# NeRF-3DTalker/NeRF-3DTalker-code

Hardware: AMD Instinct MI355X
Metric: rendered frames/sec @512^2 x 64 samples/ray (higher is better)
Workload: dtype bf16; 1 GPU; cfg2-R: 16 heads/GPU/step, 64x64 rays x 64 samples -> fused MLP+composite -> neural renderer -> 512x512 RGB (+ background image); rays_per_frame=4096, samples_per_ray=64, parallelism=frames sharded over 1 rank(s), no data-path collective, ranks_seen_by_backend=1

## Files before the change

### include/n3dt.h

```cpp
#ifndef N3DT_API_H_
#define N3DT_API_H_

#include <stddef.h>
#include <stdint.h>

#ifdef __cplusplus
extern "C" {
#endif

#define N3DT_ABI_VERSION 5

#define N3DT_F32 0
#define N3DT_BF16 1
#define N3DT_F16 2
#define N3DT_BF16X3 3

#define N3DT_OK 0
#define N3DT_EINVAL (-1)
#define N3DT_EWORKSPACE (-2)
#define N3DT_EHIP (-3)

#define N3DT_PE_DIM 63
#define N3DT_MLP_LAYERS 12

// ... 76 lines not shown

int n3dt_fine_sample(const N3dtGeom* g, int n_fine, const float* weight, const float* T, const float* t_rand, const float* u,
                     float* z_planes, void* stream);

int n3dt_sample_points(const N3dtGeom* g, const float* xy, const float* R, const float* T, const float* Kinv, const float* t_rand,
                       float* pts, float* zvals, float* z_dists, float* ray_d, float* ray_l, void* stream);
int n3dt_embed(int batch, size_t m, const float* pts, float* pe, void* stream);
int n3dt_embed_freqs(int batch, size_t m, int n_freqs, const float* pts, float* pe, void* stream);
size_t n3dt_mlp_points_workspace_bytes(const N3dtGeom* g, size_t m);
int n3dt_mlp_points(const N3dtGeom* g, size_t m, const N3dtMlpParams* p, const float* audio, const float* embed_vps,
                    const float* embed_vds, float* rgb, float* density, void* workspace, size_t workspace_bytes, void* stream);
int n3dt_composite(int batch, int n_rays, int n_samples, int channels, const float* rgb, const float* density, const float* z_dists,
                   const float* zvals, float* feat, float* bg_alpha, float* depth, float* weight, void* stream);
int n3dt_x16_pack_probe(int precision, int form, size_t n, const float* in, uint16_t* out, void* stream);
int n3dt_x16_pe_probe(int precision, int form, size_t n, const float* points, uint16_t* out, void* stream);

size_t n3dt_neural_render_workspace_bytes(const N3dtGeom* g, int nb);
int n3dt_neural_render_fwd(const N3dtGeom* g, int nb, int precision, const N3dtRenderParams* p, const float* featmap,
                           float* img, void* workspace, size_t workspace_bytes, void* stream);

int n3dt_neural_render_pack(const N3dtGeom* g, int nb, int precision, const N3dtRenderParams* p, void* workspace,
                            size_t workspace_bytes, void* stream);
int n3dt_neural_render_fwd_reuse(const N3dtGeom* g, int nb, int precision, const N3dtRenderParams* p, const float* featmap,
                                 float* img, void* workspace, size_t workspace_bytes, void* stream);
int n3dt_feat_to_rgb0(int nb, int n_pix, const float* featmap, const float* w, const float* b, float* rgb0, void* stream);
int n3dt_neural_render_fwd16_reuse(const N3dtGeom* g, int nb, int precision, const N3dtRenderParams* p, const void* featmap16,
                                   const float* rgb0, float* img, void* workspace, size_t workspace_bytes, void* stream);

size_t n3dt_render_train_saved_bytes(const N3dtGeom* g);
size_t n3dt_render_train_workspace_bytes(const N3dtGeom* g);
// ... 214 lines not shown
```

### nerf-3dtalker-code_amd/csrc/n3dt_api.hip

```cpp
#include <hip/hip_runtime.h>
#include <stdarg.h>
#include <stdio.h>
#include <stdlib.h>
#include <string.h>

#include <mutex>

#include "../../include/n3dt.h"
#include "n3dt_layout.h"
#include "n3dt_launch.h"
#include "eval_metrics_core.h"
#include "lpips_core.h"
#include "mel_core.h"
#include "syncnet_core.h"
#include "wav2lip_core.h"
#include "s3fd_core.h"

static thread_local char g_err[256] = "";

__attribute__((format(printf, 2, 3))) static int failf(int code, const char* fmt, ...) {
    va_list ap;
    va_start(ap, fmt);
    vsnprintf(g_err, sizeof(g_err), fmt, ap);
    va_end(ap);
// ... 258 lines not shown
    if (n < 512 || n % 512 != 0 || n / 512 > 0x7fffffffu) return fail(N3DT_EINVAL, "n3dt_x16_pack_probe: n must be a multiple of 512, at most 2^40");
    if (!in || !out) return fail(N3DT_EINVAL, "n3dt_x16_pack_probe: NULL argument");
    n3dt_launch_x16_pack_probe(precision, form, n, in, out, (hipStream_t)stream);
    return check_hip("n3dt_x16_pack_probe");
}

extern "C" int n3dt_x16_pe_probe(int precision, int form, size_t n, const float* points, uint16_t* out, void* stream) {
    if (precision != N3DT_BF16 && precision != N3DT_F16) return fail(N3DT_EINVAL, "n3dt_x16_pe_probe: precision must be N3DT_BF16 or N3DT_F16");
    if (form != 0 && form != 1) return fail(N3DT_EINVAL, "n3dt_x16_pe_probe: form must be 0 (by octave half) or 1 (per channel)");
    if (n < 32 || n % 32 != 0 || n / 32 > 0x7fffffffu) return fail(N3DT_EINVAL, "n3dt_x16_pe_probe: n must be a multiple of 32, at most 2^36");
    if (!points || !out) return fail(N3DT_EINVAL, "n3dt_x16_pe_probe: NULL argument");
    n3dt_launch_x16_pe_probe(precision, form, n, points, out, (hipStream_t)stream);
    return check_hip("n3dt_x16_pe_probe");
}

extern "C" int n3dt_fine_sample(const N3dtGeom* g, int n_fine, const float* weight, const float* T, const float* t_rand, const float* u,
                                float* z_planes, void* stream) {
    int rc = check_geom(g, N3DT_F32);
    if (rc) return rc;
    if (!weight || !T || !z_planes) return fail(N3DT_EINVAL, "n3dt_fine_sample: NULL argument");
    if (g->z_planes_given && !t_rand) return fail(N3DT_EINVAL, "n3dt_fine_sample: z_planes_given but no coarse planes passed as t_rand");
    if (g->n_samples < 3) return fail(N3DT_EINVAL, "n3dt_fine_sample: needs at least 3 coarse samples");
    if (n_fine < 0 || g->n_samples + n_fine + 1 > 2048) return fail(N3DT_EINVAL, "n3dt_fine_sample: more than 2048 planes per ray");
    n3dt_launch_fine_sample(g, n_fine, weight, T, t_rand, u, z_planes, (hipStream_t)stream);
    return check_hip("n3dt_fine_sample");
}

extern "C" size_t n3dt_neural_render_workspace_bytes(const N3dtGeom* g, int nb) {
    if (!g || nb < 1 || g->n_blocks < 1 || g->n_blocks > N3DT_MAX_BLOCKS || g->featmap_size < 2) return 0;
    return n3dt_nr_workspace_floats(g, nb) * sizeof(float);
// ... 887 lines not shown
```

### nerf-3dtalker-code_amd/csrc/n3dt_launch.h

```cpp
#pragma once
#include <stddef.h>
#include <hip/hip_runtime.h>

#include "../../include/n3dt.h"

struct MelSignal;

extern "C" {
int n3dt_prof_span_begin(hipStream_t s);
void n3dt_prof_span_end(int slot, hipStream_t s);

void n3dt_launch_small_gemm(int M, int N, int K, const float* A, long sam, long sak, const float* B, long sbn, long sbk, float* C, long ldc,
                            int accumulate, hipStream_t s);
void n3dt_launch_pack(const N3dtGeom* g, int precision, const N3dtMlpParams* p, void* packed, hipStream_t stream);
void n3dt_launch_fold(const N3dtGeom* g, const N3dtMlpParams* p, const float* shape, const float* appea, const float* audio, float* fold,
                      int merged_rgb, hipStream_t stream);
void n3dt_launch_rayfold(const N3dtGeom* g, const float* fold, const float* ray_bias, hipStream_t s);
void n3dt_launch_ray_vd_bias(const N3dtGeom* g, const float* w_vd, long ld_w, const float* xy, const float* R, const float* Kinv,
                             float* ray_bias, hipStream_t s);
void n3dt_launch_ray_head(const N3dtGeom* g, int bpr, int bs, const float* part, const float* wlocal, const float* tail,
                          const float* bg_featmap, int bg_hwc, float* fg_feat, float* bg_alpha, float* depth, float* weight,
                          float* merge_feat, hipStream_t stream);
void n3dt_launch_ray_head_mfma(const N3dtGeom* g, int bpr, int bs, const float* part, const float* wlocal, const float* tail,
                               const float* bg_featmap, int bg_hwc, float* fg_feat, float* bg_alpha, float* depth, float* weight,
// ... 20 lines not shown
                                    float* geo, void* gates, hipStream_t stream);
void n3dt_launch_nerf_fwd_x16s(const N3dtGeom* g, const void* packed, const float* fold, const float* xy, const float* R, const float* T,
                               const float* Kinv, const float* t_rand, float* part, float* wlocal, hipStream_t stream);

void n3dt_launch_sample_points(const N3dtGeom* g, const float* xy, const float* R, const float* T, const float* Kinv, const float* t_rand,
                               float* pts, float* zvals, float* z_dists, float* ray_d, float* ray_l, hipStream_t s);
void n3dt_launch_embed(int B, size_t M, const float* pts, float* pe, hipStream_t s);
void n3dt_launch_embed_freqs(int B, size_t M, int n_freqs, const float* pts, float* pe, hipStream_t s);
size_t n3dt_seam_mlp_ws_floats(const N3dtGeom* g, size_t M);
void n3dt_launch_mlp_points(const N3dtGeom* g, size_t M, const N3dtMlpParams* p, const float* audio, const float* vps, const float* vds,
                            float* rgb, float* density, float* ws, hipStream_t s);
void n3dt_launch_composite(int B, int Nr, int Ns, int C, const float* rgb, const float* density, const float* z_dists, const float* zvals,
                           float* feat, float* bg_alpha, float* depth, float* weight, hipStream_t s);
void n3dt_launch_x16_pe_probe(int precision, int form, size_t n, const float* points, unsigned short* out, hipStream_t s);
void n3dt_launch_x16_pack_probe(int precision, int form, size_t n, const float* in, unsigned short* out, hipStream_t s);

size_t n3dt_nr_workspace_floats(const N3dtGeom* g, int nb);
void n3dt_launch_feat_to_rgb0(int nb, int n_pix, const float* featmap, const float* w, const float* b, float* rgb0, hipStream_t s);
void n3dt_launch_neural_render16(const N3dtGeom* g, int nb, int precision, const N3dtRenderParams* p, const void* featmap16,
                                 const float* rgb0, float* img, float* ws, hipStream_t s);
void n3dt_launch_neural_render(const N3dtGeom* g, int nb, int precision, const N3dtRenderParams* p, const float* featmap, float* img,
                               float* ws, int pack_mode, hipStream_t s);
void n3dt_launch_nr_train16_fwd(const N3dtGeom* g, int nb, const N3dtRenderParams* p, const float* featmap, float* img,
                                unsigned char* saved, unsigned char* ws, hipStream_t s);
void n3dt_launch_gemm_regions_bf16(int M, int N, int K, int n_regions, const void* const* base, const int* width, const int* ld,
                                   const float* Wt, const void* gate, void* y, hipStream_t s);
void n3dt_launch_conv1x1_bwd_bf16(int M, int N, int K, const void* dy, const float* Wt, int mode, const void* res, void* y, hipStream_t s);
void n3dt_launch_conv1x1_bf16(int M, int N, int K, const void* x, int x_is_16, const float* Wt, const float* bias, float slope, void* y,
                              hipStream_t s);

// ... 109 lines not shown
```

### nerf-3dtalker-code_amd/csrc/nerf_fwd_x16.hip

```cpp
#include "x16_core.h"
#include "n3dt_launch.h"


#ifndef X16_SAVE_DEPTH
#define X16_SAVE_DEPTH 3
#endif
#ifndef X16_FWD_ISSUE
#define X16_FWD_ISSUE 0, 1, 2
#endif
template <int PREC>
struct X16SaveStage {
    unsigned char* tile0;
    unsigned* gate0;
};

enum { X16_BIAS_GLOBAL_MFMA = 0, X16_BIAS_LDS_MFMA = 1, X16_BIAS_LDS_C = 2 };
#define X16_BIAS_SLOT 1536
struct X16BiasLds {
    unsigned char* slots;
    unsigned addr;
    __device__ __forceinline__ void stage_in(const float* table, const int n, const int slot, const int lane, const int at = 0) const {
#pragma unroll
        for (int i = 0; i < 6; ++i)
            if (64 * i < n)
                __builtin_amdgcn_global_load_lds((const GLOBAL_AS void*)(table + 64 * i + lane),
                                                 (LDS_AS void*)(slots + slot * X16_BIAS_SLOT + 4 * at + 256 * i), 4, 0, 0);
    }
    __device__ __forceinline__ unsigned at(const int slot, const int at = 0) const { return addr + slot * X16_BIAS_SLOT + 4 * at; }
};
struct X16TileInit {
    f32x4 q[2][4];
    template <int SET, int OFF>
    __device__ __forceinline__ void issue(const unsigned table) {
        asm volatile("ds_read_b128 %0, %4 offset:%5\n\tds_read_b128 %1, %4 offset:%6\n\t"
                     "ds_read_b128 %2, %4 offset:%7\n\tds_read_b128 %3, %4 offset:%8"
                     : "=&v"(q[SET][0]), "=&v"(q[SET][1]), "=&v"(q[SET][2]), "=&v"(q[SET][3])
                     : "v"(table), "i"(OFF), "i"(OFF + 32), "i"(OFF + 64), "i"(OFF + 96)
                     : "memory");
    }
    template <int SET>
    __device__ __forceinline__ void landed() {
// ... 31 lines not shown
    [[maybe_unused]] float bias_cur = 0.0f, bias_nxt = 0.0f;
    if constexpr (LB) {
        x16_bias_read<0>(bias_cur, bias_lds);
        asm volatile("s_waitcnt lgkmcnt(0)" : "+v"(bias_cur));
    } else if constexpr (!CINIT) {
        bias_cur = bias[c];
    }
    auto finish_half = [&](const int t, const int half) {
        float v[8];
#pragma unroll
        for (int r = 0; r < 8; ++r) v[r] = acc[8 * half + r];
        frag f = X16<PREC>::pack(v);
        if (MODE == MODE_HIDDEN) f = X16<PREC>::relu(f, relu_lo);
        hout[2 * t + half] = f;
    };
    static_for<0, NT>([&](auto ot_c) {
        constexpr int ot = decltype(ot_c)::value;
        constexpr int cs = (PAR + ot) & 1, ns = cs ^ 1;
        constexpr bool FETCH = CINIT && ot + 1 < NT;
        X16_T(const unsigned long long s0 = x16_now();)
        if constexpr (CINIT) {
            if constexpr (ot == 0) ti.template settle<cs>();
            if constexpr (FETCH) ti.template issue<ns, (ot + 1) * 128>(bias_lds);
            acc = ti.template get<cs>();
        } else {
            const frag bf = X16<PREC>::bias_frag(bias_cur, h == 0);
            if constexpr (LB) {
                if constexpr (ot + 1 < NT) x16_bias_read<(ot + 1) * 128>(bias_nxt, bias_lds);
            } else {
                if (ot + 1 < NT) bias_cur = bias[(ot + 1) * 32 + c];
            }
            f32x16 zero;
#pragma unroll
            for (int r = 0; r < 16; ++r) zero[r] = 0.0f;
            acc = X16<PREC>::mfma(bf, ones, zero);
        }
        X16_T(const unsigned long long s1 = x16_now(); const unsigned long long rv0 = ws.t_rv;)
        static_for<0, KS>([&](auto ks_c) {
            constexpr int ks = decltype(ks_c)::value;
            const frag a_cur = ws.template next<MODE == MODE_COMPOSITE, NT * KS, ot * KS + ks,
                                                (FETCH && ks < WS::depth - 1) ? X16_TILE_INIT_READS : 0>();
            frag b;
            if (ks < KPE) {
                if (pe_lds) b = *reinterpret_cast<const frag*>(pe_lds + ks * X16_PIECE);
                else b = pe_reg[ks < 4 ? ks : 0];
            } else {
                b = hin[ks >= KPE ? ks - KPE : 0];
            }
            acc = X16<PREC>::mfma(a_cur, b, acc);
        });
        if constexpr (FETCH) ti.template landed<ns>();
        else if constexpr (CINIT && NEXT && ot + 1 == NT) ti.template issue<ns, 0>(next_lds);
        if constexpr (LB && ot + 1 < NT) {
            asm volatile("" : "+v"(bias_nxt), "+v"(acc));
            bias_cur = bias_nxt;
        }
        X16_T(const unsigned long long s2 = x16_now();)
        if (PACKS) {
            finish_half(ot, 0);
            finish_half(ot, 1);
        }
        if constexpr (SAVE && PACKS) {
#ifndef X16_DIAG_NOIMG
            x16_image_store<PREC>(hout[2 * ot], hout[2 * ot + 1], sv->tile0 + ot * 2 * X16_PIECE);
// ... 19 lines not shown
            aux = acc[0];
        } else if (MODE == MODE_COMPOSITE) {
#pragma unroll
            for (int r = 0; r < 16; ++r) red[(ot & 1) * 16 + r] = fmaxf(acc[r], 0.0f) * aux;
            if constexpr (SAVE) {
#pragma unroll
                for (int half = 0; half < 2; ++half) {
                    float v[8];
#pragma unroll
                    for (int r = 0; r < 8; ++r) v[r] = fmaxf(acc[8 * half + r], 0.0f);
                    __builtin_nontemporal_store(X16<PREC>::pack(v), reinterpret_cast<frag*>(sv->tile0 + (2 * ot + half) * X16_PIECE));
                }
                ws.note_stores(2);
            }
            if (ot & 1) {
                float s = butterfly32(red, c);
                const int v = ((c & 1) << 4) | ((c & 2) << 2) | (c & 4) | ((c & 8) >> 2) | ((c & 16) >> 4);
                const int reg = v & 15, tile = (ot - 1) + (v >> 4);
                if (live) po[tile * 32 + (reg & 3) + 8 * (reg >> 2) + 4 * h] = s;
            }
        }
        X16_T(const unsigned long long s3 = x16_now(); ws.t_bias += s1 - s0; ws.t_mfma += (s2 - s1) - (ws.t_rv - rv0); ws.t_epi += s3 - s2;
              if (ws.tl && ws.tile_no >= 20 && ws.tile_no < 33 && (threadIdx.x & 63) == 0) {
                  ws.tl[4 + 2 * (ws.tile_no - 20)] = (float)(s1 & 0xFFFFFF);
                  ws.tl[5 + 2 * (ws.tile_no - 20)] = (float)(s2 & 0xFFFFFF);
              }
              ++ws.tile_no;)
    });
}

struct X16TrainSave {
    unsigned char* xT;
    unsigned char* gS;
    float* geo;
    unsigned* gates;
};

template <int PREC, int WAVES, bool SAVE = false>
__device__ __forceinline__ void nerf_fwd_x16_body(
    const N3dtGeom& g, const unsigned char* __restrict__ packed, const float* __restrict__ fold, const float* __restrict__ xy,
    const float* __restrict__ R, const float* __restrict__ T, const float* __restrict__ Kinv, const float* __restrict__ t_rand,
    float* __restrict__ part, float* __restrict__ wlocal, int bpr, long total_blocks, unsigned char* lds, const int wave,
    const X16TrainSave tsv = X16TrainSave{nullptr, nullptr, nullptr, nullptr}) {
    typedef typename X16<PREC>::frag frag;
    const int lane = threadIdx.x & 63;
    const int c = lane & 31, h = lane >> 5;
    X16_T(const unsigned long long t_entry = x16_now();)

    typedef WeightStream<PREC, WAVES, X16_NCHUNK, X16_NBUF, SAVE ? X16_SAVE_DEPTH : X16_DEPTH,
                         std::conditional_t<SAVE, X16Issue<>, X16Issue<X16_FWD_ISSUE>>> WS;
    WS ws;
    if constexpr (SAVE) {
        ws.gsrc = packed + (size_t)wave * WS::PPW * X16_PIECE + lane * 16;
    } else {
        ws.gsrc = packed + (size_t)wave * WS::PPW * X16_PIECE;
        ws.voff = lane * 16;
    }
    ws.ring = lds;
    ws.lds_addr0 = (unsigned)(size_t)(LDS_AS unsigned char*)lds + lane * 16;
// ... 31 lines not shown
    auto sv_hidden = [&](const int l) -> const X16SaveStage<PREC>* {
        if constexpr (SAVE) {
            svs.tile0 = xT_blk + (size_t)(2 + 12 * l) * 2 * X16_PIECE;
            svs.gate0 = tsv.gates + ((size_t)rec * 8 + l) * 6 * 64 + lane;
            return &svs;
        } else {
            return nullptr;
        }
    };
    constexpr int BIAS = SAVE ? X16_BIAS_LDS_MFMA : X16_BIAS_LDS_C;
    constexpr int BIAS_DEN = BIAS == X16_BIAS_LDS_C ? X16_BIAS_LDS_C : X16_BIAS_GLOBAL_MFMA;
    X16BiasLds bl{nullptr, 0u};
    constexpr int DEN_AT = 192;
    bl.slots = lds + X16_NBUF * X16_CH * X16_PIECE + (size_t)WAVES * 4 * X16_PIECE + (size_t)wave * 2 * X16_BIAS_SLOT;
    bl.addr = (unsigned)(size_t)(LDS_AS unsigned char*)bl.slots + (BIAS == X16_BIAS_LDS_C ? 16 * h : 4 * c);
    bl.stage_in(fb + n3dt_bias_offset(0), 384, 0, lane);
    auto bias_slot = [&](const int k) -> unsigned {
        if (k < 7) {
            bl.stage_in(fb + n3dt_bias_offset(k + 1), 384, (k + 1) & 1, lane);
        } else {
            bl.stage_in(b10, 192, 0, lane);
            if constexpr (BIAS_DEN == X16_BIAS_LDS_C) bl.stage_in(fb + n3dt_bias_offset(8), 64, 0, lane, DEN_AT);
        }
        return bl.at(k & 1);
    };
    if constexpr (!SAVE) pe_settle(pe);
    ws.prologue_wait();
    X16_T(const unsigned long long t_head = x16_now() - t_entry;)
    X16_T(if (wlocal && live) ws.tl = wlocal + (size_t)blk * X16_BS;)
    X16TileInit ti;
    if constexpr (BIAS == X16_BIAS_LDS_C) ti.template issue<0, 0>(bl.at(0));

    frag ha[24], hb[24];
    float aux;
    x16_stage<PREC, WAVES, 4, 4, 12, MODE_HIDDEN, SAVE, BIAS, 0, true>(ws, ti, fb + n3dt_bias_offset(0), bias_slot(0), bl.at(1), pe, nullptr, ha, ha, aux, po, live, lane, sv_hidden(0));
    x16_stage<PREC, WAVES, 24, 0, 12, MODE_HIDDEN, SAVE, BIAS, 0, true>(ws, ti, fb + n3dt_bias_offset(1), bias_slot(1), bl.at(0), pe, nullptr, ha, hb, aux, po, live, lane, sv_hidden(1));
    x16_stage<PREC, WAVES, 24, 0, 12, MODE_HIDDEN, SAVE, BIAS, 0, true>(ws, ti, fb + n3dt_bias_offset(2), bias_slot(2), bl.at(1), pe, nullptr, hb, ha, aux, po, live, lane, sv_hidden(2));
    x16_stage<PREC, WAVES, 24, 0, 12, MODE_HIDDEN, SAVE, BIAS, 0, true>(ws, ti, fb + n3dt_bias_offset(3), bias_slot(3), bl.at(0), pe, nullptr, ha, hb, aux, po, live, lane, sv_hidden(3));
    x16_stage<PREC, WAVES, 24, 0, 12, MODE_HIDDEN, SAVE, BIAS, 0, true>(ws, ti, fb + n3dt_bias_offset(4), bias_slot(4), bl.at(1), pe, nullptr, hb, ha, aux, po, live, lane, sv_hidden(4));
    x16_stage<PREC, WAVES, 28, 4, 12, MODE_HIDDEN, SAVE, BIAS, 0, true>(ws, ti, fb + n3dt_bias_offset(5), bias_slot(5), bl.at(0), pe, pe_lds, ha, hb, aux, po, live, lane, sv_hidden(5));
    x16_stage<PREC, WAVES, 24, 0, 12, MODE_HIDDEN, SAVE, BIAS, 0, true>(ws, ti, fb + n3dt_bias_offset(6), bias_slot(6), bl.at(1), pe, nullptr, hb, ha, aux, po, live, lane, sv_hidden(6));
    x16_stage<PREC, WAVES, 24, 0, 12, MODE_HIDDEN, SAVE, BIAS, 0, true>(ws, ti, fb + n3dt_bias_offset(7), bias_slot(7), bl.at(0, DEN_AT), pe, nullptr, ha, hb, aux, po, live, lane, sv_hidden(7));
    x16_stage<PREC, WAVES, 24, 0, 1, MODE_DENSITY, false, BIAS_DEN, 0, true>(ws, ti, fb + n3dt_bias_offset(8), bl.at(0, DEN_AT), bl.at(0), pe, nullptr, hb, ha, aux, po, live, lane);
    {
        float sp = __shfl(aux, c, 64);
        if constexpr (SAVE) {
            if (live && h == 0) {
                tsv.geo[(size_t)blk * 64 + c] = sp;
                tsv.geo[(size_t)blk * 64 + 32 + c] = dist;
            }
        }
        float sigma = fmaxf(sp, 0.0f);
        float alpha = 1.0f - expf(-sigma * dist);
        float x = 1.0f - alpha + 1e-10f;
        float Tl = n3dt_exclusive_prod<32>(x, c);
        float w = alpha * Tl;
        float s0 = w, s1 = w * zval;
#pragma unroll
        for (int off = 16; off > 0; off >>= 1) {
            s0 += __shfl_xor(s0, off, 32);
            s1 += __shfl_xor(s1, off, 32);
        }
        float tprod = __shfl(Tl * x, 31, 32);
        if (live && lane == 0) {
            po[N3DT_G + 0] = s0;
            po[N3DT_G + 1] = s1;
            po[N3DT_G + 2] = tprod;
            po[N3DT_G + 3] = 0.0f;
        }
#ifndef X16_STAMP
        if (live && wlocal && h == 0) wlocal[(size_t)blk * X16_BS + c] = w;
#endif
        aux = w;
    }
    if constexpr (SAVE) {
        svs.tile0 = tsv.gS + (size_t)rec * 12 * X16_PIECE + lane * 16;
        svs.gate0 = nullptr;
    }
// ... 74 lines not shown
```

### nerf-3dtalker-code_amd/csrc/seams.hip

```cpp
#include "gemm32.h"
#include "n3dt_device.h"
#include "x16_core.h"
#include "n3dt_launch.h"

__global__ void seam_sample_kernel(N3dtGeom g, const float* __restrict__ xy, const float* __restrict__ R, const float* __restrict__ T,
                                   const float* __restrict__ Kinv, const float* __restrict__ t_rand, float* __restrict__ pts,
                                   float* __restrict__ zvals, float* __restrict__ z_dists, float* __restrict__ ray_d,
                                   float* __restrict__ ray_l) {
    const size_t total = (size_t)g.batch * g.n_rays * g.n_samples;
    const size_t i = (size_t)blockIdx.x * blockDim.x + threadIdx.x;
    if (i >= total) return;
    const int s = (int)(i % g.n_samples);
    const size_t rg = i / g.n_samples;
    const int ray = (int)(rg % g.n_rays), b = (int)(rg / g.n_rays);
    float p[3], dist, zval;
    n3dt_sample_point(g, xy, R, T, Kinv, t_rand, b, ray, s, p, dist, zval);
    const size_t M = (size_t)g.n_rays * g.n_samples, m = (size_t)ray * g.n_samples + s;
    if (pts)
#pragma unroll
        for (int d = 0; d < 3; ++d) pts[((size_t)b * 3 + d) * M + m] = p[d];
    if (zvals) zvals[(size_t)b * M + m] = zval;
    if (z_dists) z_dists[(size_t)b * M + m] = dist;
    if (s == 0 && (ray_d || ray_l)) {
        const float x = xy[(int64_t)b * g.xy_stride_b + (int64_t)ray * g.xy_stride_r];
// ... 271 lines not shown
        if (form == 0) hipLaunchKernelGGL((x16_pe_probe_kernel<N3DT_F16, 0>), grid, block, 0, s, n, points, out);
        else hipLaunchKernelGGL((x16_pe_probe_kernel<N3DT_F16, 1>), grid, block, 0, s, n, points, out);
    }
}

extern "C" void n3dt_launch_x16_pack_probe(int precision, int form, size_t n, const float* in, unsigned short* out, hipStream_t s) {
    const dim3 grid((unsigned)(n / 512)), block(64);
    if (precision == N3DT_BF16) {
        if (form == 0) hipLaunchKernelGGL((x16_pack_probe_kernel<N3DT_BF16, 0>), grid, block, 0, s, n, in, out);
        else hipLaunchKernelGGL((x16_pack_probe_kernel<N3DT_BF16, 1>), grid, block, 0, s, n, in, out);
    } else {
        if (form == 0) hipLaunchKernelGGL((x16_pack_probe_kernel<N3DT_F16, 0>), grid, block, 0, s, n, in, out);
        else hipLaunchKernelGGL((x16_pack_probe_kernel<N3DT_F16, 1>), grid, block, 0, s, n, in, out);
    }
}
```

### nerf-3dtalker-code_amd/csrc/x16_core.h

```cpp
#pragma once
#include <stdlib.h>

#include <type_traits>

#include "n3dt_device.h"
#include "n3dt_layout.h"

typedef __bf16 bf16x8 __attribute__((ext_vector_type(8)));
typedef __bf16 x16_bf16x2 __attribute__((ext_vector_type(2)));
typedef _Float16 x16_f16x2 __attribute__((ext_vector_type(2)));
typedef float x16_f32x2 __attribute__((ext_vector_type(2)));
typedef unsigned x16_u32x2 __attribute__((ext_vector_type(2)));
typedef unsigned x16_u32x4 __attribute__((ext_vector_type(4)));

#define X16_BS 32
#define X16_CH 24
#define X16_PIECE 1024
#define X16_NCHUNK (2280 / X16_CH)
#define X16_XT_TILES 98
#define GLOBAL_AS __attribute__((address_space(1)))
#define LDS_AS __attribute__((address_space(3)))

template <int PREC>
__device__ __forceinline__ unsigned x16_cvt2(const float a, const float b) {
// ... 425 lines not shown
#pragma unroll
    for (int step = 1; step < 5; ++step) {
        const int m = 16 >> step;
        const bool bit = (c & m) != 0;
        const int n = 32 >> step;
#pragma unroll
        for (int i = 0; i < n / 2; ++i) {
            float keep = bit ? v[2 * i + 1] : v[2 * i];
            float send = bit ? v[2 * i] : v[2 * i + 1];
            v[i] = keep + __shfl_xor(send, m, 64);
        }
    }
    return v[0];
}

__device__ __forceinline__ int x16_image_lane_offset(const int lane) { return 64 * (lane & 31) + 16 * (lane >> 5); }
template <int PREC>
__device__ __forceinline__ void x16_image_store(const typename X16<PREC>::frag f0, const typename X16<PREC>::frag f1, unsigned char* dst) {
    typedef typename X16<PREC>::frag frag;
#if X16_NT_STORE
    __builtin_nontemporal_store(f0, reinterpret_cast<frag*>(dst));
    __builtin_nontemporal_store(f1, reinterpret_cast<frag*>(dst + 32));
#else
    *reinterpret_cast<frag*>(dst) = f0;
    *reinterpret_cast<frag*>(dst + 32) = f1;
#endif
}
__device__ __forceinline__ unsigned x16_tr_lane_offset(const int lane) {
    const int r = lane & 31, h = lane >> 5, q = (r & 15) >> 2, p = r & 3;
    return 64u * (8 * h + q) + 32u * (r >> 4) + 8u * ((p & 1) * 2 + (p >> 1));
// ... 29 lines not shown
```

### nerf-3dtalker-code_amd/n3dt/_lib.py

```python
import ctypes
import os

_HERE = os.path.dirname(os.path.abspath(__file__))
LIB_PATH = os.environ.get("N3DT_LIB") or os.path.join(os.path.dirname(_HERE), "lib", "libn3dt.so")

F32, BF16, F16, BF16X3 = 0, 1, 2, 3
PRECISIONS = {"fp32": F32, "f32": F32, "bf16": BF16, "fp16": F16, "f16": F16, "bf16x3": BF16X3}
MLP_LAYERS = 12
MAX_BLOCKS = 8

MLP_ORDER = ["FeaExt_module_%d" % i for i in range(8)] + ["density_module", "RGB_layer_0", "RGB_layer_1", "RGB_layer_2"]


class Geom(ctypes.Structure):
    _fields_ = [
        ("batch", ctypes.c_int32), ("n_rays", ctypes.c_int32), ("n_samples", ctypes.c_int32),
        ("hidden", ctypes.c_int32), ("feat_nc", ctypes.c_int32), ("shape_dim", ctypes.c_int32),
        ("appea_dim", ctypes.c_int32), ("audio_dim", ctypes.c_int32), ("featmap_size", ctypes.c_int32),
        ("n_blocks", ctypes.c_int32), ("world_z1", ctypes.c_float), ("world_z2", ctypes.c_float),
        ("xy_stride_b", ctypes.c_int64), ("xy_stride_c", ctypes.c_int64), ("xy_stride_r", ctypes.c_int64),
        ("z_planes_given", ctypes.c_int32), ("bg_is_hwc", ctypes.c_int32), ("vd_dim", ctypes.c_int32),
    ]


# ... 137 lines not shown
        "n3dt_vgg_workspace_bytes": (sz, [ci, ci, ci]),
        "n3dt_vgg_loss_fwd": (ci, [ci, ci, ci, vp, vp, vp, vp, f32, vp, vp, sz, vp, sz, vp]),
        "n3dt_vgg_loss_bwd": (ci, [ci, ci, ci, vp, vp, vp, vp, sz, vp, vp, sz, vp]),
        "n3dt_vgg_conv_stage": (ci, [ci, vp, ci, ci, ci, ci, ci, vp, vp, vp, ci, vp]),
        "n3dt_a2s_saved_bytes": (sz, [ci]),
        "n3dt_a2s_workspace_bytes": (sz, [ci]),
        "n3dt_a2s_fwd": (ci, [ci, a2p, vp, vp, vp, vp, vp, vp, sz, vp, sz, vp]),
        "n3dt_a2s_bwd": (ci, [ci, a2p, vp, vp, sz, vp, vp, sz, vp]),
        "n3dt_flat_adam_record_bytes": (sz, [ci]),
        "n3dt_flat_adam_step": (ci, [vp, vp, ci, vp, ci, vp, vp]),
        "n3dt_render_fwd16": (ci, [gp, ci, vp, mp] + [vp] * 19 + [vp, sz, vp]),
        "n3dt_neural_render_fwd16_reuse": (ci, [gp, ci, ci, rp, vp, vp, vp, vp, sz, vp]),
        "n3dt_feat_to_rgb0": (ci, [ci, ci, vp, vp, vp, vp, vp]),
        "n3dt_x16_pack_probe": (ci, [ci, ci, sz, vp, vp, vp]),
        "n3dt_x16_pe_probe": (ci, [ci, ci, sz, vp, vp, vp]),
        "n3dt_eval_metrics_workspace_bytes": (sz, [ci, ci, ci]),
        "n3dt_eval_metrics": (ci, [ci, ci, ci, vp, vp, vp, vp, vp, sz, vp]),
        "n3dt_lpips_packed_bytes": (sz, []),
        "n3dt_lpips_pack": (ci, [ctypes.POINTER(LpipsParams), vp, vp]),
        "n3dt_lpips_workspace_bytes": (sz, [ci, ci, ci]),
        "n3dt_lpips": (ci, [ci, ci, ci, ci, vp, vp, vp, vp, vp, vp, sz, vp]),
        "n3dt_mel_workspace_bytes": (sz, []),
        "n3dt_mel_spectrogram": (ci, [i64, vp, i64, vp, i64, i64, ci, vp, vp, vp, i64, ci, vp, sz, vp]),
        "n3dt_mel_windows": (ci, [i64, vp, i64, ci, ci, vp, vp, vp]),
        "n3dt_syncnet_packed_bytes": (sz, []),
        "n3dt_syncnet_pack": (ci, [ctypes.POINTER(SyncnetParams), vp, vp]),
        "n3dt_syncnet_workspace_bytes": (sz, [ci]),
        "n3dt_syncnet_face_windows": (ci, [ci, ci, ci, vp, vp, ci, vp, vp]),
        "n3dt_syncnet_fwd": (ci, [ci, vp, vp, vp, vp, vp, ci, ci, ci, vp, vp, vp, vp, sz, vp]),
        "n3dt_syncnet_block": (ci, [ci, ci, vp, vp, vp, vp, sz, vp]),
# ... 69 lines not shown
```

### nerf-3dtalker-code_amd/n3dt/ops.py

```python
import ctypes

import torch

from . import _lib
from ._lib import Geom, MlpParams, RenderParams, check, lib


def _stream():
    return ctypes.c_void_p(torch.cuda.current_stream().cuda_stream)


def _ptr(t):
    if t is None:
        return None
    assert t.is_cuda, "libn3dt works on device memory only (no CPU fallback)"
    return ctypes.c_void_p(t.data_ptr())


def _f32c(t):
    return t.detach().to(dtype=torch.float32).contiguous()


class _Workspace:

# ... 156 lines not shown
def x16_pack_probe(x, precision, form=0):
    x = _f32c(x)
    prec = _lib.PRECISIONS[precision] if isinstance(precision, str) else int(precision)
    out = torch.empty(x.shape, dtype=torch.bfloat16 if prec == _lib.BF16 else torch.float16, device=x.device)
    check(lib().n3dt_x16_pack_probe(prec, int(form), x.numel(), _ptr(x), _ptr(out), _stream()), "n3dt_x16_pack_probe")
    return out


def x16_pe_probe(points, precision, form=0):
    points = _f32c(points)
    assert points.dim() == 2 and points.shape[1] == 3, "points must be [n, 3]"
    n = points.shape[0]
    prec = _lib.PRECISIONS[precision] if isinstance(precision, str) else int(precision)
    out = torch.empty((n // 32, 4, 64, 8), dtype=torch.bfloat16 if prec == _lib.BF16 else torch.float16, device=points.device)
    check(lib().n3dt_x16_pe_probe(prec, int(form), n, _ptr(points), _ptr(out), _stream()), "n3dt_x16_pe_probe")
    return out


def ray_vd_bias(geom, w_rgb1, xy, R, Kinv, out=None):
    assert w_rgb1.is_contiguous() and w_rgb1.dim() == 2 and w_rgb1.shape[0] == 192 and w_rgb1.shape[1] >= 384 + 27
    B, Nr = geom.batch, geom.n_rays
    rb = out if out is not None else torch.empty(B, Nr, 192, dtype=torch.float32, device=xy.device)
    w_vd = ctypes.c_void_p(w_rgb1.data_ptr() + 384 * 4)
    check(lib().n3dt_ray_vd_bias(ctypes.byref(geom), w_vd, int(w_rgb1.shape[1]), _ptr(xy), _ptr(R), _ptr(Kinv), _ptr(rb), _stream()),
          "n3dt_ray_vd_bias")
    return rb


def mlp_points(geom, params, audio, embed_vps, embed_vds):
    vps, vds = _f32c(embed_vps), _f32c(embed_vds)
# ... 207 lines not shown
```

Before: 2214 frames/s.

## Use DPP/permlane cross-lane ops, prefetch PE fragments, and scalar-addressed bias staging

Replaces the LDS-backed shuffles (ds_bpermute) in the forward fused MLP+composite kernel's butterfly reduction, transmittance prefix product, and sums with DPP row ops and v_permlane16/32_swap. It also software-pipelines the positional-encoding B-fragment reads one k-step ahead with explicit wait counts. Bias table staging now uses a scalar base address plus a per-lane offset. The aim is to take LDS traffic and VGPR address math out of the MFMA loop; the hand-tuned wait counts and inline asm add correctness risk. A probe kernel is added to validate the new cross-lane primitives against the old ones.

```diff
diff --git a/include/n3dt.h b/include/n3dt.h
--- a/include/n3dt.h
+++ b/include/n3dt.h
@@ -114,6 +114,7 @@
                    const float* zvals, float* feat, float* bg_alpha, float* depth, float* weight, void* stream);
 int n3dt_x16_pack_probe(int precision, int form, size_t n, const float* in, uint16_t* out, void* stream);
 int n3dt_x16_pe_probe(int precision, int form, size_t n, const float* points, uint16_t* out, void* stream);
+int n3dt_x16_reduce_probe(int form, int n_waves, const float* in, float* out, void* stream);
 
 size_t n3dt_neural_render_workspace_bytes(const N3dtGeom* g, int nb);
 int n3dt_neural_render_fwd(const N3dtGeom* g, int nb, int precision, const N3dtRenderParams* p, const float* featmap,
diff --git a/nerf-3dtalker-code_amd/csrc/n3dt_api.hip b/nerf-3dtalker-code_amd/csrc/n3dt_api.hip
--- a/nerf-3dtalker-code_amd/csrc/n3dt_api.hip
+++ b/nerf-3dtalker-code_amd/csrc/n3dt_api.hip
@@ -296,6 +296,14 @@
     return check_hip("n3dt_x16_pe_probe");
 }
 
+extern "C" int n3dt_x16_reduce_probe(int form, int n_waves, const float* in, float* out, void* stream) {
+    if (form != 0 && form != 1) return fail(N3DT_EINVAL, "n3dt_x16_reduce_probe: form must be 0 (LDS crossbar) or 1 (vector ALU)");
+    if (n_waves < 1) return fail(N3DT_EINVAL, "n3dt_x16_reduce_probe: n_waves must be positive");
+    if (!in || !out) return fail(N3DT_EINVAL, "n3dt_x16_reduce_probe: NULL argument");
+    n3dt_launch_x16_reduce_probe(form, n_waves, in, out, (hipStream_t)stream);
+    return check_hip("n3dt_x16_reduce_probe");
+}
+
 extern "C" int n3dt_fine_sample(const N3dtGeom* g, int n_fine, const float* weight, const float* T, const float* t_rand, const float* u,
                                 float* z_planes, void* stream) {
     int rc = check_geom(g, N3DT_F32);
diff --git a/nerf-3dtalker-code_amd/csrc/n3dt_launch.h b/nerf-3dtalker-code_amd/csrc/n3dt_launch.h
--- a/nerf-3dtalker-code_amd/csrc/n3dt_launch.h
+++ b/nerf-3dtalker-code_amd/csrc/n3dt_launch.h
@@ -58,6 +58,7 @@
                            float* feat, float* bg_alpha, float* depth, float* weight, hipStream_t s);
 void n3dt_launch_x16_pe_probe(int precision, int form, size_t n, const float* points, unsigned short* out, hipStream_t s);
 void n3dt_launch_x16_pack_probe(int precision, int form, size_t n, const float* in, unsigned short* out, hipStream_t s);
+void n3dt_launch_x16_reduce_probe(int form, int n_waves, const float* in, float* out, hipStream_t s);
 
 size_t n3dt_nr_workspace_floats(const N3dtGeom* g, int nb);
 void n3dt_launch_feat_to_rgb0(int nb, int n_pix, const float* featmap, const float* w, const float* b, float* rgb0, hipStream_t s);
diff --git a/nerf-3dtalker-code_amd/csrc/nerf_fwd_x16.hip b/nerf-3dtalker-code_amd/csrc/nerf_fwd_x16.hip
--- a/nerf-3dtalker-code_amd/csrc/nerf_fwd_x16.hip
+++ b/nerf-3dtalker-code_amd/csrc/nerf_fwd_x16.hip
@@ -2,11 +2,25 @@
 #include "n3dt_launch.h"
 
 
+#ifndef X16_STAMP_TILE0
+#define X16_STAMP_TILE0 60
+#endif
 #ifndef X16_SAVE_DEPTH
 #define X16_SAVE_DEPTH 3
 #endif
 #ifndef X16_FWD_ISSUE
 #define X16_FWD_ISSUE 0, 1, 2
+#endif
+#ifndef X16_XLANE_VALU
+#define X16_XLANE_VALU 1
+#endif
+template <bool SAVE>
+using X16FwdXlane = std::conditional_t<X16_XLANE_VALU != 0 && !SAVE, X16XlaneValu, X16XlaneLds>;
+#ifndef X16_SKIP_COUNTED
+#define X16_SKIP_COUNTED 1
+#endif
+#ifndef X16_BIAS_SCALAR
+#define X16_BIAS_SCALAR 1
 #endif
 template <int PREC>
 struct X16SaveStage {
@@ -25,6 +39,17 @@
             if (64 * i < n)
                 __builtin_amdgcn_global_load_lds((const GLOBAL_AS void*)(table + 64 * i + lane),
                                                  (LDS_AS void*)(slots + slot * X16_BIAS_SLOT + 4 * at + 256 * i), 4, 0, 0);
+    }
+    template <int N>
+    __device__ __forceinline__ void stage_in_scalar(const float* table, const int slot, unsigned& lane4, const int at = 0) const {
+        static_assert(N % 64 == 0, "whole 256-byte rows");
+        static_for<0, N / 64>([&](auto i_c) {
+            constexpr int I = decltype(i_c)::value;
+            unsigned long long b = (unsigned long long)(table + 64 * I);
+            asm volatile("" : "+s"(b), "+v"(lane4));
+            __builtin_amdgcn_global_load_lds((const GLOBAL_AS void*)((const GLOBAL_AS unsigned char*)b + lane4),
+                                             (LDS_AS void*)(slots + slot * X16_BIAS_SLOT + 4 * at + 256 * I), 4, 0, 0);
+        });
     }
     __device__ __forceinline__ unsigned at(const int slot, const int at = 0) const { return addr + slot * X16_BIAS_SLOT + 4 * at; }
 };
@@ -86,13 +111,24 @@
         if (MODE == MODE_HIDDEN) f = X16<PREC>::relu(f, relu_lo);
         hout[2 * t + half] = f;
     };
+    constexpr bool PE_ASM = X16_SKIP_COUNTED && !SAVE && KPE > 0 && KS > KPE;
+    [[maybe_unused]] frag pb[2];
+    [[maybe_unused]] const unsigned pe_addr = PE_ASM ? (unsigned)(size_t)(LDS_AS const unsigned char*)pe_lds : 0u;
+    if constexpr (PE_ASM) {
+        static_assert(CINIT && KS - 1 > KPE, "the first tile's PE0 is covered by the stage's settle; PE0 of the next tile goes out at the last k-step");
+        static_assert(WS::depth <= 3, "three reads are younger than PE(ks) at its wait, and next<>() allows depth - 1 + EXTRA");
+        ws.template read_frag<0>(pb[0], pe_addr);
+    }
     static_for<0, NT>([&](auto ot_c) {
         constexpr int ot = decltype(ot_c)::value;
         constexpr int cs = (PAR + ot) & 1, ns = cs ^ 1;
         constexpr bool FETCH = CINIT && ot + 1 < NT;
         X16_T(const unsigned long long s0 = x16_now();)
         if constexpr (CINIT) {
-            if constexpr (ot == 0) ti.template settle<cs>();
+            if constexpr (ot == 0) {
+                ti.template settle<cs>();
+                if constexpr (PE_ASM) asm volatile("" : "+v"(pb[0]));
+            }
             if constexpr (FETCH) ti.template issue<ns, (ot + 1) * 128>(bias_lds);
             acc = ti.template get<cs>();
         } else {
@@ -110,16 +146,31 @@
         X16_T(const unsigned long long s1 = x16_now(); const unsigned long long rv0 = ws.t_rv;)
         static_for<0, KS>([&](auto ks_c) {
             constexpr int ks = decltype(ks_c)::value;
-            const frag a_cur = ws.template next<MODE == MODE_COMPOSITE, NT * KS, ot * KS + ks,
-                                                (FETCH && ks < WS::depth - 1) ? X16_TILE_INIT_READS : 0>();
+            constexpr int bias_extra = (FETCH && ks < WS::depth - 1) ? X16_TILE_INIT_READS : 0;
             frag b;
-            if (ks < KPE) {
-                if (pe_lds) b = *reinterpret_cast<const frag*>(pe_lds + ks * X16_PIECE);
-                else b = pe_reg[ks < 4 ? ks : 0];
+            if constexpr (PE_ASM) {
+                constexpr bool ahead = ks + 1 < KPE, wrap = ks == KS - 1 && ot + 1 < NT;
+                if constexpr (ahead) ws.template read_frag<(ks + 1) * X16_PIECE>(pb[(ks + 1) & 1], pe_addr);
+                if constexpr (wrap) ws.template read_frag<0>(pb[0], pe_addr);
+                constexpr int extra = ((ahead || wrap) ? 1 : 0) + (ks == 0 ? bias_extra : ks < KPE ? 0 : bias_extra);
+                const frag a_cur = ws.template next<MODE == MODE_COMPOSITE, NT * KS, ot * KS + ks, extra>();
+                if constexpr (ks < KPE) {
+                    asm volatile("" : "+v"(pb[ks & 1]));
+                    b = pb[ks & 1];
+                } else {
+                    b = hin[ks - KPE];
+                }
+                acc = X16<PREC>::mfma(a_cur, b, acc);
             } else {
-                b = hin[ks >= KPE ? ks - KPE : 0];
-            }
-            acc = X16<PREC>::mfma(a_cur, b, acc);
+                const frag a_cur = ws.template next<MODE == MODE_COMPOSITE, NT * KS, ot * KS + ks, bias_extra>();
+                if (ks < KPE) {
+                    if (pe_lds) b = *reinterpret_cast<const frag*>(pe_lds + ks * X16_PIECE);
+                    else b = pe_reg[ks < 4 ? ks : 0];
+                } else {
+                    b = hin[ks >= KPE ? ks - KPE : 0];
+                }
+                acc = X16<PREC>::mfma(a_cur, b, acc);
+            }
         });
         if constexpr (FETCH) ti.template landed<ns>();
         else if constexpr (CINIT && NEXT && ot + 1 == NT) ti.template issue<ns, 0>(next_lds);
@@ -169,16 +220,16 @@
                 ws.note_stores(2);
             }
             if (ot & 1) {
-                float s = butterfly32(red, c);
+                float s = X16FwdXlane<SAVE>::butterfly(red, c);
                 const int v = ((c & 1) << 4) | ((c & 2) << 2) | (c & 4) | ((c & 8) >> 2) | ((c & 16) >> 4);
                 const int reg = v & 15, tile = (ot - 1) + (v >> 4);
                 if (live) po[tile * 32 + (reg & 3) + 8 * (reg >> 2) + 4 * h] = s;
             }
         }
         X16_T(const unsigned long long s3 = x16_now(); ws.t_bias += s1 - s0; ws.t_mfma += (s2 - s1) - (ws.t_rv - rv0); ws.t_epi += s3 - s2;
-              if (ws.tl && ws.tile_no >= 20 && ws.tile_no < 33 && (threadIdx.x & 63) == 0) {
-                  ws.tl[4 + 2 * (ws.tile_no - 20)] = (float)(s1 & 0xFFFFFF);
-                  ws.tl[5 + 2 * (ws.tile_no - 20)] = (float)(s2 & 0xFFFFFF);
+              if (ws.tl && ws.tile_no >= X16_STAMP_TILE0 && ws.tile_no < X16_STAMP_TILE0 + 13 && (threadIdx.x & 63) == 0) {
+                  ws.tl[4 + 2 * (ws.tile_no - X16_STAMP_TILE0)] = (float)(s1 & 0xFFFFFF);
+                  ws.tl[5 + 2 * (ws.tile_no - X16_STAMP_TILE0)] = (float)(s2 & 0xFFFFFF);
               }
               ++ws.tile_no;)
     });
@@ -198,6 +249,7 @@
     float* __restrict__ part, float* __restrict__ wlocal, int bpr, long total_blocks, unsigned char* lds, const int wave,
     const X16TrainSave tsv = X16TrainSave{nullptr, nullptr, nullptr, nullptr}) {
     typedef typename X16<PREC>::frag frag;
+    typedef X16FwdXlane<SAVE> XL;
     const int lane = threadIdx.x & 63;
     const int c = lane & 31, h = lane >> 5;
     X16_T(const unsigned long long t_entry = x16_now();)
@@ -259,13 +311,19 @@
     constexpr int DEN_AT = 192;
     bl.slots = lds + X16_NBUF * X16_CH * X16_PIECE + (size_t)WAVES * 4 * X16_PIECE + (size_t)wave * 2 * X16_BIAS_SLOT;
     bl.addr = (unsigned)(size_t)(LDS_AS unsigned char*)bl.slots + (BIAS == X16_BIAS_LDS_C ? 16 * h : 4 * c);
-    bl.stage_in(fb + n3dt_bias_offset(0), 384, 0, lane);
+    [[maybe_unused]] unsigned lane4 = lane * 4;
+    auto stage_table = [&](auto n_c, const float* table, const int slot, const int at) {
+        constexpr int N = decltype(n_c)::value;
+        if constexpr (X16_BIAS_SCALAR && !SAVE) bl.template stage_in_scalar<N>(table, slot, lane4, at);
+        else bl.stage_in(table, N, slot, lane, at);
+    };
+    stage_table(std::integral_constant<int, 384>{}, fb + n3dt_bias_offset(0), 0, 0);
     auto bias_slot = [&](const int k) -> unsigned {
         if (k < 7) {
-            bl.stage_in(fb + n3dt_bias_offset(k + 1), 384, (k + 1) & 1, lane);
+            stage_table(std::integral_constant<int, 384>{}, fb + n3dt_bias_offset(k + 1), (k + 1) & 1, 0);
         } else {
-            bl.stage_in(b10, 192, 0, lane);
-            if constexpr (BIAS_DEN == X16_BIAS_LDS_C) bl.stage_in(fb + n3dt_bias_offset(8), 64, 0, lane, DEN_AT);
+            stage_table(std::integral_constant<int, 192>{}, b10, 0, 0);
+            if constexpr (BIAS_DEN == X16_BIAS_LDS_C) stage_table(std::integral_constant<int, 64>{}, fb + n3dt_bias_offset(8), 0, DEN_AT);
         }
         return bl.at(k & 1);
     };
@@ -288,7 +346,7 @@
     x16_stage<PREC, WAVES, 24, 0, 12, MODE_HIDDEN, SAVE, BIAS, 0, true>(ws, ti, fb + n3dt_bias_offset(7), bias_slot(7), bl.at(0, DEN_AT), pe, nullptr, ha, hb, aux, po, live, lane, sv_hidden(7));
     x16_stage<PREC, WAVES, 24, 0, 1, MODE_DENSITY, false, BIAS_DEN, 0, true>(ws, ti, fb + n3dt_bias_offset(8), bl.at(0, DEN_AT), bl.at(0), pe, nullptr, hb, ha, aux, po, live, lane);
     {
-        float sp = __shfl(aux, c, 64);
+        float sp = XL::from_lower(aux, c);
         if constexpr (SAVE) {
             if (live && h == 0) {
                 tsv.geo[(size_t)blk * 64 + c] = sp;
@@ -298,15 +356,11 @@
         float sigma = fmaxf(sp, 0.0f);
         float alpha = 1.0f - expf(-sigma * dist);
         float x = 1.0f - alpha + 1e-10f;
-        float Tl = n3dt_exclusive_prod<32>(x, c);
+        float Tl = XL::excl_prod(x, c);
         float w = alpha * Tl;
         float s0 = w, s1 = w * zval;
-#pragma unroll
-        for (int off = 16; off > 0; off >>= 1) {
-            s0 += __shfl_xor(s0, off, 32);
-            s1 += __shfl_xor(s1, off, 32);
-        }
-        float tprod = __shfl(Tl * x, 31, 32);
+        XL::sum32x2(s0, s1);
+        float tprod = XL::from_last(Tl * x);
         if (live && lane == 0) {
             po[N3DT_G + 0] = s0;
             po[N3DT_G + 1] = s1;
diff --git a/nerf-3dtalker-code_amd/csrc/seams.hip b/nerf-3dtalker-code_amd/csrc/seams.hip
--- a/nerf-3dtalker-code_amd/csrc/seams.hip
+++ b/nerf-3dtalker-code_amd/csrc/seams.hip
@@ -309,3 +309,26 @@
         else hipLaunchKernelGGL((x16_pack_probe_kernel<N3DT_F16, 1>), grid, block, 0, s, n, in, out);
     }
 }
+
+template <class XL>
+__global__ void __launch_bounds__(64) x16_reduce_probe_kernel(const float* __restrict__ in, float* __restrict__ out) {
+    const int lane = threadIdx.x, c = lane & 31;
+    const float* src = in + (size_t)blockIdx.x * 36 * 64 + lane;
+    float* dst = out + (size_t)blockIdx.x * 6 * 64 + lane;
+    float v[32];
+#pragma unroll
+    for (int r = 0; r < 32; ++r) v[r] = src[64 * r];
+    const float x = src[64 * 32], a = src[64 * 33], b = src[64 * 34], aux = src[64 * 35];
+    dst[0] = XL::butterfly(v, c);
+    dst[64] = XL::excl_prod(x, c);
+    dst[128] = XL::sum32(a);
+    dst[192] = XL::sum32(b);
+    dst[256] = XL::from_lower(aux, c);
+    dst[320] = XL::from_last(x);
+}
+
+extern "C" void n3dt_launch_x16_reduce_probe(int form, int n_waves, const float* in, float* out, hipStream_t s) {
+    const dim3 grid((unsigned)n_waves), block(64);
+    if (form == 0) hipLaunchKernelGGL((x16_reduce_probe_kernel<X16XlaneLds>), grid, block, 0, s, in, out);
+    else hipLaunchKernelGGL((x16_reduce_probe_kernel<X16XlaneValu>), grid, block, 0, s, in, out);
+}
diff --git a/nerf-3dtalker-code_amd/csrc/x16_core.h b/nerf-3dtalker-code_amd/csrc/x16_core.h
--- a/nerf-3dtalker-code_amd/csrc/x16_core.h
+++ b/nerf-3dtalker-code_amd/csrc/x16_core.h
@@ -463,6 +463,113 @@
     return v[0];
 }
 
+struct X16XlaneLds {
+    static __device__ __forceinline__ float butterfly(float (&v)[32], const int c) { return butterfly32(v, c); }
+    static __device__ __forceinline__ float excl_prod(const float x, const int c) { return n3dt_exclusive_prod<32>(x, c); }
+    static __device__ __forceinline__ float sum32(float s) {
+#pragma unroll
+        for (int off = 16; off > 0; off >>= 1) s += __shfl_xor(s, off, 32);
+        return s;
+    }
+    static __device__ __forceinline__ void sum32x2(float& s0, float& s1) {
+#pragma unroll
+        for (int off = 16; off > 0; off >>= 1) {
+            s0 += __shfl_xor(s0, off, 32);
+            s1 += __shfl_xor(s1, off, 32);
+        }
+    }
+    static __device__ __forceinline__ float from_lower(const float v, const int c) { return __shfl(v, c, 64); }
+    static __device__ __forceinline__ float from_last(const float v) { return __shfl(v, 31, 32); }
+};
+struct X16XlaneValu {
+    template <int M>
+    static __device__ __forceinline__ float row_xor(const float v) {
+        const int i = __builtin_bit_cast(int, v);
+        int r;
+        if constexpr (M == 8) {
+            r = __builtin_amdgcn_update_dpp(i, i, 0x128, 0xf, 0xf, false);
+        } else if constexpr (M == 4) {
+            r = __builtin_amdgcn_update_dpp(i, i, 0x104, 0xf, 0x5, false);
+            r = __builtin_amdgcn_update_dpp(r, i, 0x114, 0xf, 0xa, false);
+        } else if constexpr (M == 2) {
+            r = __builtin_amdgcn_update_dpp(i, i, 0x4e, 0xf, 0xf, false);
+        } else {
+            static_assert(M == 1, "partner inside the row");
+            r = __builtin_amdgcn_update_dpp(i, i, 0xb1, 0xf, 0xf, false);
+        }
+        return __builtin_bit_cast(float, r);
+    }
+    static __device__ __forceinline__ void row_pairs(const float v, float& a, float& b) {
+        a = v;
+        b = v;
+        asm("s_nop 1\n\tv_permlane16_swap_b32 %0, %1\n\ts_nop 1" : "+v"(a), "+v"(b));
+    }
+    static __device__ __forceinline__ float butterfly(float (&v)[32], const int c) {
+#pragma unroll
+        for (int i = 0; i < 16; ++i) {
+            float a = v[2 * i], b = v[2 * i + 1];
+            asm("s_nop 1\n\tv_permlane16_swap_b32 %0, %1\n\ts_nop 1" : "+v"(a), "+v"(b));
+            v[i] = a + b;
+        }
+        static_for<1, 5>([&](auto step_c) {
+            constexpr int step = decltype(step_c)::value, m = 16 >> step, n = 32 >> step;
+            const bool bit = (c & m) != 0;
+#pragma unroll
+            for (int i = 0; i < n / 2; ++i) {
+                const float keep = bit ? v[2 * i + 1] : v[2 * i];
+                const float send = bit ? v[2 * i] : v[2 * i + 1];
+                v[i] = keep + row_xor<m>(send);
+            }
+        });
+        return v[0];
+    }
+    template <int OFF>
+    static __device__ __forceinline__ float up(const float v) {
+        float lo, hi;
+        row_pairs(v, lo, hi);
+        if constexpr (OFF == 16) {
+            return lo;
+        } else {
+            const int below = __builtin_amdgcn_update_dpp(0, __builtin_bit_cast(int, lo), 0x120 + OFF, 0xf, 0xf, false);
+            return __builtin_bit_cast(float, __builtin_amdgcn_update_dpp(below, __builtin_bit_cast(int, v), 0x110 + OFF, 0xf, 0xf, false));
+        }
+    }
+    static __device__ __forceinline__ float excl_prod(const float x, const int c) {
+        float incl = x;
+        static_for<0, 5>([&](auto k_c) {
+            constexpr int off = 1 << decltype(k_c)::value;
+            const float o = up<off>(incl);
+            if (c >= off) incl *= o;
+        });
+        const float excl = up<1>(incl);
+        return c == 0 ? 1.0f : excl;
+    }
+    static __device__ __forceinline__ float sum32(float s) {
+        float a, b;
+        row_pairs(s, a, b);
+        s = a + b;
+        s += row_xor<8>(s);
+        s += row_xor<4>(s);
+        s += row_xor<2>(s);
+        s += row_xor<1>(s);
+        return s;
+    }
+    static __device__ __forceinline__ void sum32x2(float& s0, float& s1) {
+        s0 = sum32(s0);
+        s1 = sum32(s1);
+    }
+    static __device__ __forceinline__ float from_lower(const float v, const int) {
+        float a = v, b = v;
+        asm("s_nop 1\n\tv_permlane32_swap_b32 %0, %1\n\ts_nop 1" : "+v"(a), "+v"(b));
+        return a;
+    }
+    static __device__ __forceinline__ float from_last(const float v) {
+        const int i = __builtin_bit_cast(int, v);
+        const int lo = __builtin_amdgcn_readlane(i, 31), hi = __builtin_amdgcn_readlane(i, 63);
+        return __builtin_bit_cast(float, (int)(threadIdx.x & 32) ? hi : lo);
+    }
+};
+
 __device__ __forceinline__ int x16_image_lane_offset(const int lane) { return 64 * (lane & 31) + 16 * (lane >> 5); }
 template <int PREC>
 __device__ __forceinline__ void x16_image_store(const typename X16<PREC>::frag f0, const typename X16<PREC>::frag f1, unsigned char* dst) {
diff --git a/nerf-3dtalker-code_amd/n3dt/_lib.py b/nerf-3dtalker-code_amd/n3dt/_lib.py
--- a/nerf-3dtalker-code_amd/n3dt/_lib.py
+++ b/nerf-3dtalker-code_amd/n3dt/_lib.py
@@ -175,6 +175,7 @@
         "n3dt_feat_to_rgb0": (ci, [ci, ci, vp, vp, vp, vp, vp]),
         "n3dt_x16_pack_probe": (ci, [ci, ci, sz, vp, vp, vp]),
         "n3dt_x16_pe_probe": (ci, [ci, ci, sz, vp, vp, vp]),
+        "n3dt_x16_reduce_probe": (ci, [ci, ci, vp, vp, vp]),
         "n3dt_eval_metrics_workspace_bytes": (sz, [ci, ci, ci]),
         "n3dt_eval_metrics": (ci, [ci, ci, ci, vp, vp, vp, vp, vp, sz, vp]),
         "n3dt_lpips_packed_bytes": (sz, []),
diff --git a/nerf-3dtalker-code_amd/n3dt/ops.py b/nerf-3dtalker-code_amd/n3dt/ops.py
--- a/nerf-3dtalker-code_amd/n3dt/ops.py
+++ b/nerf-3dtalker-code_amd/n3dt/ops.py
@@ -194,6 +194,14 @@
     prec = _lib.PRECISIONS[precision] if isinstance(precision, str) else int(precision)
     out = torch.empty((n // 32, 4, 64, 8), dtype=torch.bfloat16 if prec == _lib.BF16 else torch.float16, device=points.device)
     check(lib().n3dt_x16_pe_probe(prec, int(form), n, _ptr(points), _ptr(out), _stream()), "n3dt_x16_pe_probe")
+    return out
+
+
+def x16_reduce_probe(x, form=0):
+    x = _f32c(x)
+    assert x.dim() == 3 and x.shape[1:] == (36, 64), "x must be [n_waves, 36, 64]"
+    out = torch.empty((x.shape[0], 6, 64), dtype=torch.float32, device=x.device)
+    check(lib().n3dt_x16_reduce_probe(int(form), x.shape[0], _ptr(x), _ptr(out), _stream()), "n3dt_x16_reduce_probe")
     return out
 
 
```

Result: no change. 2231 frames/s (median of 6 runs) (+0.8%).
